# zju3dv/NeuralRecon-W

Measured on NVIDIA H100. Metric: training rays/sec, higher is better.
Workload: dtype bf16 (3-product split forward, plain bf16 backward, fp32 accumulate)

## Files before the change

neuralrecon-w_b200/csrc/engine.cu:

```cuda
#include <stdlib.h>

#include "engine.h"

namespace nrw {

static constexpr float INV_SQRT2 = 0.70710678118654752440f;

struct Carver {
  char* base;
  long long off = 0;
  bool dry;
  void* take(long long bytes) {
    off = round_up(off, 1024);
    void* p = dry ? nullptr : base + off;
    off += bytes;
    return p;
  }
  float* f32(long long n) { return reinterpret_cast<float*>(take(n * 4)); }
  Planes planes(long long rows, int ld, int P) {
    const long long ps = round_up(rows * ld, 512);
    bf16* p = reinterpret_cast<bf16*>(take(ps * P * 2));
    return Planes{p, ps, ld};
  }
};
// ... 51 lines not shown
  c.use_nerf_slot(0);
  c.fwd_cached = false;
  c.ge_acc = cv.f32(4);
  if (with_bwd) {
    const int PB = c.bwd_planes > 0 ? c.bwd_planes : P;
    c.DQ0 = cv.planes(M, 64, PB);
    c.DQodd = cv.planes(M, 512, PB);
    c.DQeven = cv.planes(M, 512, PB);
    c.DQ4 = cv.planes(M, 512, PB);
    c.DA[0] = cv.planes(M, 512, PB);
    c.DA[1] = cv.planes(M, 512, PB);
    c.DFEAT = cv.planes(M, 512, PB);
    c.DQ8f = cv.f32(M * 512);
    for (int l = 0; l < 8; ++l)
      c.DA2[l] = c.aux_bf16 ? side_bf16(reinterpret_cast<bf16*>(cv.take(M * 512 * 2)), 512) : side_f32(cv.f32(M * 512), 512);
    c.dX[0] = cv.planes(M, 256, PB);
    c.dX[1] = cv.planes(M, 256, PB);
    c.dH2 = cv.planes(M, 128, PB);
    c.dH1 = cv.planes(M, 128, PB);
    c.dXF = cv.planes(M, 512, PB);
    c.dNA[0] = cv.planes(M, 128, PB);
    c.dNA[1] = cv.planes(M, 128, PB);
    c.dNF = cv.planes(M, 256, PB);
    c.dNH[0] = cv.planes(M, 256, PB);
    c.dNH[1] = cv.planes(M, 256, PB);
    c.tail = cv.f32(M * 128);
    c.c_dn = cv.f32(M * 3);
    c.c_ddens = cv.f32(M);
    c.gs = cv.f32(c.pm.grad_floats);
  }
  const long long RT = (long long)max_rays * max_T;
  for (int i = 0; i < 2; ++i) { c.gz[i] = cv.f32(RT); c.gsdf[i] = cv.f32(RT); }
  c.gznew = cv.f32(RT);
  c.gsdfnew = cv.f32(RT);
  c.gcdf = cv.f32(RT);
  c.gorder = reinterpret_cast<int32_t*>(cv.f32(RT));
  c.g_pts = cv.f32(RT * 3);
  if (with_bwd) {
    c.g_dsdf = cv.f32(RT);
    c.g_dnrm = cv.f32(RT * 3);
    c.g_drgb = cv.f32(RT * 3);
    c.g_dbga = cv.f32(RT);
    c.g_dbgc = cv.f32(RT * 3);
  }
}

long long workspace_bytes(const nrw_ctx& c0, int chunk_rows, int with_bwd, int max_rays, int max_T, int n_slots_sdf,
                          int n_slots_nerf) {
  nrw_ctx c = c0;
  Carver cv{nullptr, 0, true};
  carve(c, cv, chunk_rows, with_bwd, max_rays, max_T, n_slots_sdf < 1 ? 1 : n_slots_sdf, n_slots_nerf < 1 ? 1 : n_slots_nerf);
  return round_up(cv.off, 1024) + 1024;
}

int carve_workspace(nrw_ctx& c, void* base, long long bytes, int chunk_rows, int with_bwd, int max_rays,
                    int max_T, int n_slots_sdf, int n_slots_nerf, cudaStream_t s) {
  NRW_CHECK(chunk_rows >= 128 && chunk_rows % 128 == 0, NRW_ERR_ARG, "chunk_rows=%d must be a multiple of 128", chunk_rows);
  NRW_CHECK((reinterpret_cast<uintptr_t>(base) & 255) == 0, NRW_ERR_ARG, "workspace must be 256B aligned");
  if (n_slots_sdf < 1) n_slots_sdf = 1;
  if (n_slots_nerf < 1) n_slots_nerf = 1;
  const long long need = workspace_bytes(c, chunk_rows, with_bwd, max_rays, max_T, n_slots_sdf, n_slots_nerf);
  NRW_CHECK(bytes >= need, NRW_ERR_WORKSPACE, "workspace too small: %lld < %lld bytes", bytes, need);
  char* b = reinterpret_cast<char*>((reinterpret_cast<uintptr_t>(base) + 1023) & ~uintptr_t(1023));
  Carver cv{b, 0, false};
  carve(c, cv, chunk_rows, with_bwd, max_rays, max_T, n_slots_sdf, n_slots_nerf);
  NRW_CUDA_OK(cudaMemsetAsync(b, 0, cv.off, s));
  c.Mc = chunk_rows; c.with_bwd = with_bwd; c.max_rays = max_rays; c.max_T = max_T;
  c.bound = true;
  return NRW_OK;
}

static int mm(nrw_ctx& c, Planes A, Planes B, int M, int N, int K, Epi e, cudaStream_t s) {
  GemmDesc g;
  g.A = A; g.B = B; g.n_planes = c.cur_planes; g.M = M; g.N = N; g.K = K; g.mn_major = 0; g.k_slices = 1;
  if (e.out_pl.p) e.n_planes = c.cur_planes;
  g.epi = e;
  return gemm(c.backend, g, s);
}
static int mm_dw(nrw_ctx& c, Planes dY, Planes X, int M, int layer, cudaStream_t s) {
  const PackedLayer& L = c.pm.layers[layer];
  GemmDesc g;
  g.A = dY; g.B = X; g.n_planes = c.cur_planes;
  g.M = L.Np; g.N = L.Kp; g.K = M; g.mn_major = 1;
  const int tiles = cdiv(g.M, 128) * cdiv(g.N, gemm_tc_tile_n(g.N));
  int dev = 0, n_sm = 0;
  NRW_CUDA_OK(cudaGetDevice(&dev));
  NRW_CUDA_OK(cudaDeviceGetAttribute(&n_sm, cudaDevAttrMultiProcessorCount, dev));
  int ks = 2 * n_sm / tiles;
  const int max_ks = M / 512 > 0 ? M / 512 : 1;
  if (ks > max_ks) ks = max_ks;
  if (ks < 1) ks = 1;
  const int kb_total = cdiv(M, 64);
  const int kb_per = cdiv(kb_total, ks);
  ks = cdiv(kb_total, kb_per);
  g.k_slices = ks;
  Epi e;
  e.out_f32 = c.dW(layer); e.ld_f32 = L.Kp; e.atomic = 1;
  g.epi = e;
  return gemm(c.backend, g, s);
}
static int bias_grad(nrw_ctx& c, Planes dY, int M, int layer, cudaStream_t s) {
  return launch_colsum(dY, c.cur_planes, nullptr, 0, M, c.pm.layers[layer].Np, nullptr, c.db(layer), nullptr, s);
}
static void gate_from(nrw_ctx& c, Epi& e, int l, int planes) {
  e.aux_u = c.U[l + 1];
  e.aux_u_planes = planes;
  e.aux_u_scale = (l == 3) ? 1.41421356237309504880f : 1.0f;
}
static Planes rows(Planes P, int r0) { return Planes{P.p + (long long)r0 * P.ld, P.pstride, P.ld}; }

static bool sdf_fused_enabled(const nrw_ctx& c) {
  static const int fused_chain = getenv("NRW_SDF_FUSED") ? atoi(getenv("NRW_SDF_FUSED")) : 1;
  return fused_chain && c.backend == NRW_GEMM_TCGEN05 && c.n_planes == 2;
}
static int sdf_fused_query(nrw_ctx& c, const float* pts, int M, float* sdf, cudaStream_t s) {
  SdfFusedDesc d;
  d.pts = pts; d.sdf = sdf; d.M = M;
  for (int l = 0; l < 8; ++l) { d.W[l] = c.W(L_SDF0 + l); d.bias[l] = c.bias(L_SDF0 + l); }
  d.head_w = c.f_area + c.pm.heads.sdf_w0;
  d.head_b = c.f_area + c.pm.heads.sdf_b0;
  return sdf_fused_forward(d, s);
}

int sdf_chunk_forward(nrw_ctx& c, int M, const float* pts, bool need_normal, bool need_feat, cudaStream_t s) {
  c.cur_planes = c.n_planes;
  const int P = c.n_planes;
  NRW_TRY(launch_sdf_embed(pts, M, P, c.U0, c.U[4], s));
  const float* w0 = c.f_area + c.pm.heads.sdf_w0;
  const float* b0 = c.f_area + c.pm.heads.sdf_b0;
  const bool fused_head = !need_normal && !need_feat && M >= 256 && c.backend == NRW_GEMM_TCGEN05;
  if (fused_head && sdf_fused_enabled(c)) return sdf_fused_query(c, pts, M, c.c_sdf, s);
  for (int l = 0; l < 8; ++l) {
    Epi e;
    e.bias = c.bias(L_SDF0 + l);
    e.act = ACT_SOFTPLUS100;
    if (l == 7 && fused_head) { e.head_w = w0; e.head_partial = c.HP; }
    else e.out_pl = c.U[l + 1];
    if (l == 3) { e.scale = INV_SQRT2; e.n_store = 473; }
    NRW_TRY(mm(c, l == 0 ? c.U0 : c.U[l], c.W(L_SDF0 + l), M, 512, l == 0 ? 64 : 512, e, s));
  }
  if (fused_head) NRW_TRY(launch_sdf_head_sum(c.HP, M, b0, c.c_sdf, s));
  else NRW_TRY(launch_sdf_head(c.U[8], M, w0, b0, c.c_sdf, P, need_normal ? c.G[7] : Planes{nullptr, 0, 0}, s));
  if (need_feat) {
    Epi e;
    e.bias = c.bias(L_SDF8F);
    e.out_pl = c.FEAT;
    NRW_TRY(mm(c, c.U[8], c.W(L_SDF8F), M, 512, 512, e, s));
  }
  if (need_normal) {
    for (int l = 7; l >= 1; --l) {
      Epi e;
      e.out_pre = c.Q[l];
      gate_from(c, e, l - 1, c.n_planes);
      e.out_pl = c.G[l - 1];
      if (l == 4) { e.scale = INV_SQRT2; e.n_store = 473; }
      NRW_TRY(mm(c, c.G[l], c.WT(L_SDF0 + l), M, 512, 512, e, s));
    }
    Epi e;
    e.out_pre = c.Q[0];
    NRW_TRY(mm(c, c.G[0], c.WT(L_SDF0), M, 64, 512, e, s));
    NRW_TRY(launch_sdf_normal(pts, c.Q[0].f32(), c.Q[4].f32(), M, c.c_nrm, s));
  }
  return NRW_OK;
}

int color_chunk_forward(nrw_ctx& c, int M, const float* pts, const float* dirs, const float* a, int rows_per_src,
                        cudaStream_t s) {
  c.cur_planes = c.n_planes;
  const int P = c.n_planes;
  NRW_TRY(launch_color_embed(dirs, a, c.n_a, rows_per_src, pts, c.c_nrm, M, P, c.IN1, c.IN2, s));
  { Epi e; e.bias = c.bias(L_CX); e.out_pl = c.IN1; NRW_TRY(mm(c, c.FEAT, c.W(L_CX), M, 512, 512, e, s)); }
  { Epi e; e.bias = c.bias(L_CS0); e.act = ACT_RELU; e.out_pl = c.H1; NRW_TRY(mm(c, c.IN1, c.W(L_CS0), M, 128, 640, e, s)); }
  { Epi e; e.bias = c.bias(L_CS1); e.act = ACT_RELU; e.out_pl = c.IN2; NRW_TRY(mm(c, c.H1, c.W(L_CS1), M, 128, 128, e, s)); }
  { Epi e; e.bias = c.bias(L_CL0); e.act = ACT_RELU; e.out_pl = c.X[1]; NRW_TRY(mm(c, c.IN2, c.W(L_CL0), M, 256, 192, e, s)); }
  for (int l = 1; l <= 3; ++l) {
    Epi e; e.bias = c.bias(L_CL0 + l); e.act = ACT_RELU; e.out_pl = c.X[l + 1];
    NRW_TRY(mm(c, c.X[l], c.W(L_CL0 + l), M, 256, 256, e, s));
  }
  NRW_TRY(launch_head(3, c.X[4], P, 256, M, c.f_area + c.pm.heads.cl4_w, c.f_area + c.pm.heads.cl4_b, ACT_SIGMOID,
                      nullptr, c.c_rgb, nullptr, s));
  return NRW_OK;
// ... 320 lines not shown
```

neuralrecon-w_b200/csrc/gemm.h:

```cpp
#pragma once
#include "epilogue.cuh"

namespace nrw {

struct GemmDesc {
  Planes A;
  Planes B;
  int n_planes = 1;
  int M = 0, N = 0, K = 0;
  int mn_major = 0;
  int k_slices = 1;
  Epi epi;
};

int gemm_tc(const GemmDesc& g, cudaStream_t stream);
int gemm_simt(const GemmDesc& g, cudaStream_t stream);

inline int gemm(int backend, const GemmDesc& g, cudaStream_t stream) {
  return backend == NRW_GEMM_SIMT ? gemm_simt(g, stream) : gemm_tc(g, stream);
}

inline int n_products(int n_planes) { return n_planes == 1 ? 1 : (n_planes == 2 ? 3 : 6); }

struct SdfFusedDesc {
  const float* pts = nullptr;
  float* sdf = nullptr;
  int M = 0;
  Planes W[8];
  const float* bias[8] = {nullptr, nullptr, nullptr, nullptr, nullptr, nullptr, nullptr, nullptr};
  const float* head_w = nullptr;
  const float* head_b = nullptr;
};
int sdf_fused_forward(const SdfFusedDesc& d, cudaStream_t stream);

long long gemm_tc_launch_count();
inline int gemm_tc_tile_n(int N) { return N <= 64 ? 64 : 128; }
void gemm_tc_set_profile_buffer(unsigned long long* buf);
void gemm_tc_timing_enable(bool on);
int gemm_tc_timing_read(double* ms, double* flops, double* mma_flops, long long* launches, double* bytes);

}
```

neuralrecon-w_b200/csrc/gemm_tc.cu:

```cuda
#include <stdlib.h>

#include <mutex>
#include <unordered_map>
#include <vector>
#include <algorithm>
#include <stdio.h>

#include "gemm.h"
#include "epilogue_fast.cuh"

namespace nrw {

static constexpr int BM = 128;
static constexpr int BK = 64;
static constexpr int RING_BYTES = 192 * 1024;
static constexpr int MAX_STAGES = 8;
static constexpr int N_CONSUMER_WARPS = 8;
static constexpr int N_THREADS = 32 * N_CONSUMER_WARPS + 128;
static constexpr int PRODUCER_REGS = 40, CONSUMER_REGS = 232;
static constexpr int EPI_COLS = 64;
static constexpr int EPI_WG_BYTES = 64 * EPI_COLS * 4;
static constexpr int CS_BYTES = 1024;
static constexpr int BAR_TURN = 4;
static_assert(PRODUCER_REGS * 128 + CONSUMER_REGS * 32 * N_CONSUMER_WARPS <= 65536, "register file");
static constexpr int BAR_BYTES = 256;
static constexpr int SMEM_BYTES = 1024 + RING_BYTES + BAR_BYTES + 2 * EPI_WG_BYTES + CS_BYTES;
static_assert(SMEM_BYTES <= 232448, "dynamic shared memory limit of sm_90");

__device__ __forceinline__ int epi_swz(int r) { return ((r & 1) << 2) | (r & 2) | ((r >> 2) & 1); }

struct TcParams {
  CUtensorMap tmA[3];
  CUtensorMap tmB[3];
  int M, N, K;
  int n_planes;
  int k_slices;
  int m_tiles, n_tiles;
  Epi epi;
  unsigned long long* prof;
};
#define NRW_PROF_T0(cond) const long long _t0 = (cond) ? clock64() : 0
#define NRW_PROF_ADD(cond, slot) \
  if (cond) atomicAdd(&p.prof[blockIdx.x * 16 + (slot)], (unsigned long long)(clock64() - _t0))

__device__ __forceinline__ uint32_t smem_u32(const void* p) {
  return static_cast<uint32_t>(__cvta_generic_to_shared(p));
}
__device__ __forceinline__ void mbar_init(uint32_t bar, uint32_t count) {
  asm volatile("mbarrier.init.shared::cta.b64 [%0], %1;" ::"r"(bar), "r"(count));
}
__device__ __forceinline__ void mbar_wait(uint32_t bar, uint32_t parity) {
  asm volatile(
      "{\n"
      ".reg .pred p;\n"
      "WAIT_LOOP:\n"
      "mbarrier.try_wait.parity.shared::cta.b64 p, [%0], %1;\n"
      "@p bra.uni WAIT_DONE;\n"
      "bra.uni WAIT_LOOP;\n"
      "WAIT_DONE:\n"
      "}\n" ::"r"(bar),
      "r"(parity)
      : "memory");
}
__device__ __forceinline__ void mbar_arrive(uint32_t bar) {
  asm volatile("mbarrier.arrive.shared::cta.b64 _, [%0];" ::"r"(bar) : "memory");
}
__device__ __forceinline__ void mbar_arrive_expect_tx(uint32_t bar, uint32_t bytes) {
  asm volatile("mbarrier.arrive.expect_tx.shared::cta.b64 _, [%0], %1;" ::"r"(bar), "r"(bytes)
               : "memory");
}
__device__ __forceinline__ void tma_load_2d(uint32_t dst, const CUtensorMap* map, uint32_t bar,
                                            int x, int y) {
  asm volatile(
      "cp.async.bulk.tensor.2d.shared::cluster.global.mbarrier::complete_tx::bytes"
      " [%0], [%1, {%3, %4}], [%2];" ::"r"(dst),
      "l"(reinterpret_cast<uint64_t>(map)), "r"(bar), "r"(x), "r"(y)
      : "memory");
}
__device__ __forceinline__ void tma_prefetch_desc(const CUtensorMap* map) {
  asm volatile("prefetch.tensormap [%0];" ::"l"(reinterpret_cast<uint64_t>(map)) : "memory");
}
__device__ __forceinline__ void pdl_wait() { asm volatile("griddepcontrol.wait;" ::: "memory"); }
__device__ __forceinline__ void pdl_launch_dependents() { asm volatile("griddepcontrol.launch_dependents;" ::: "memory"); }
__device__ __forceinline__ void named_bar_sync(int id, int n) { asm volatile("bar.sync %0, %1;" ::"r"(id), "r"(n) : "memory"); }
__device__ __forceinline__ void named_bar_arrive(int id, int n) { asm volatile("bar.arrive %0, %1;" ::"r"(id), "r"(n) : "memory"); }
template <int R>
__device__ __forceinline__ void setmaxnreg_inc() { asm volatile("setmaxnreg.inc.sync.aligned.u32 %0;" ::"n"(R)); }
template <int R>
__device__ __forceinline__ void setmaxnreg_dec() { asm volatile("setmaxnreg.dec.sync.aligned.u32 %0;" ::"n"(R)); }
__device__ __forceinline__ void fence_proxy_async_smem() { asm volatile("fence.proxy.async.shared::cta;" ::: "memory"); }

__device__ __forceinline__ uint64_t make_gdesc(uint32_t saddr, uint32_t lbo_bytes, uint32_t sbo_bytes) {
  uint64_t d = 0;
  d |= (uint64_t)((saddr & 0x3FFFF) >> 4);
  d |= (uint64_t)((lbo_bytes >> 4) & 0x3FFF) << 16;
  d |= (uint64_t)((sbo_bytes >> 4) & 0x3FFF) << 32;
  d |= (uint64_t)1 << 62;
  return d;
}
__device__ __forceinline__ void wgmma_fence() { asm volatile("wgmma.fence.sync.aligned;" ::: "memory"); }
__device__ __forceinline__ void wgmma_commit() { asm volatile("wgmma.commit_group.sync.aligned;" ::: "memory"); }
template <int N>
__device__ __forceinline__ void wgmma_wait() { asm volatile("wgmma.wait_group.sync.aligned %0;" ::"n"(N) : "memory"); }
template <int N>
__device__ __forceinline__ void acc_fence(float (&d)[N]) {
#pragma unroll
  for (int i = 0; i < N; ++i) asm volatile("" : "+f"(d[i])::"memory");
}

template <int BN, int TA, int TB>
__device__ __forceinline__ void wgmma_bf16(float (&d)[BN / 2], uint64_t da, uint64_t db, uint32_t accumulate);

template <>
__device__ __forceinline__ void wgmma_bf16<64, 0, 0>(float (&d)[32], uint64_t da, uint64_t db, uint32_t accumulate) {
  asm volatile(
      "{\n.reg .pred p;\nsetp.ne.b32 p, %34, 0;\n"
      "wgmma.mma_async.sync.aligned.m64n64k16.f32.bf16.bf16 "
      "{%0, %1, %2, %3, %4, %5, %6, %7, %8, %9, %10, %11, %12, %13, %14, %15, %16, %17, %18, %19, %20, %21, %22, %23, %24, %25, "
      "%26, %27, %28, %29, %30, %31}, %32, %33, p, 1, 1, 0, 0;\n}\n"
      : "+f"(d[0]), "+f"(d[1]), "+f"(d[2]), "+f"(d[3]), "+f"(d[4]), "+f"(d[5]), "+f"(d[6]), "+f"(d[7]), "+f"(d[8]), "+f"(d[9]),
        "+f"(d[10]), "+f"(d[11]), "+f"(d[12]), "+f"(d[13]), "+f"(d[14]), "+f"(d[15]), "+f"(d[16]), "+f"(d[17]), "+f"(d[18]),
        "+f"(d[19]), "+f"(d[20]), "+f"(d[21]), "+f"(d[22]), "+f"(d[23]), "+f"(d[24]), "+f"(d[25]), "+f"(d[26]), "+f"(d[27]),
        "+f"(d[28]), "+f"(d[29]), "+f"(d[30]), "+f"(d[31])
      : "l"(da), "l"(db), "r"(accumulate));
}
template <>
__device__ __forceinline__ void wgmma_bf16<64, 1, 1>(float (&d)[32], uint64_t da, uint64_t db, uint32_t accumulate) {
  asm volatile(
      "{\n.reg .pred p;\nsetp.ne.b32 p, %34, 0;\n"
      "wgmma.mma_async.sync.aligned.m64n64k16.f32.bf16.bf16 "
      "{%0, %1, %2, %3, %4, %5, %6, %7, %8, %9, %10, %11, %12, %13, %14, %15, %16, %17, %18, %19, %20, %21, %22, %23, %24, %25, "
      "%26, %27, %28, %29, %30, %31}, %32, %33, p, 1, 1, 1, 1;\n}\n"
      : "+f"(d[0]), "+f"(d[1]), "+f"(d[2]), "+f"(d[3]), "+f"(d[4]), "+f"(d[5]), "+f"(d[6]), "+f"(d[7]), "+f"(d[8]), "+f"(d[9]),
        "+f"(d[10]), "+f"(d[11]), "+f"(d[12]), "+f"(d[13]), "+f"(d[14]), "+f"(d[15]), "+f"(d[16]), "+f"(d[17]), "+f"(d[18]),
        "+f"(d[19]), "+f"(d[20]), "+f"(d[21]), "+f"(d[22]), "+f"(d[23]), "+f"(d[24]), "+f"(d[25]), "+f"(d[26]), "+f"(d[27]),
        "+f"(d[28]), "+f"(d[29]), "+f"(d[30]), "+f"(d[31])
      : "l"(da), "l"(db), "r"(accumulate));
}
#define NRW_WGMMA_N128(TA, TB)                                                                                                          \
  template <>                                                                                                                           \
  __device__ __forceinline__ void wgmma_bf16<128, TA, TB>(float (&d)[64], uint64_t da, uint64_t db, uint32_t accumulate) {              \
    asm volatile(                                                                                                                       \
        "{\n.reg .pred p;\nsetp.ne.b32 p, %66, 0;\n"                                                                                    \
        "wgmma.mma_async.sync.aligned.m64n128k16.f32.bf16.bf16 "                                                                        \
        "{%0, %1, %2, %3, %4, %5, %6, %7, %8, %9, %10, %11, %12, %13, %14, %15, %16, %17, %18, %19, %20, %21, %22, %23, %24, %25, "    \
        "%26, %27, %28, %29, %30, %31, %32, %33, %34, %35, %36, %37, %38, %39, %40, %41, %42, %43, %44, %45, %46, %47, %48, %49, %50, " \
        "%51, %52, %53, %54, %55, %56, %57, %58, %59, %60, %61, %62, %63}, %64, %65, p, 1, 1, " #TA ", " #TB ";\n}\n"                   \
        : "+f"(d[0]), "+f"(d[1]), "+f"(d[2]), "+f"(d[3]), "+f"(d[4]), "+f"(d[5]), "+f"(d[6]), "+f"(d[7]), "+f"(d[8]), "+f"(d[9]),     \
          "+f"(d[10]), "+f"(d[11]), "+f"(d[12]), "+f"(d[13]), "+f"(d[14]), "+f"(d[15]), "+f"(d[16]), "+f"(d[17]), "+f"(d[18]),        \
          "+f"(d[19]), "+f"(d[20]), "+f"(d[21]), "+f"(d[22]), "+f"(d[23]), "+f"(d[24]), "+f"(d[25]), "+f"(d[26]), "+f"(d[27]),        \
          "+f"(d[28]), "+f"(d[29]), "+f"(d[30]), "+f"(d[31]), "+f"(d[32]), "+f"(d[33]), "+f"(d[34]), "+f"(d[35]), "+f"(d[36]),        \
          "+f"(d[37]), "+f"(d[38]), "+f"(d[39]), "+f"(d[40]), "+f"(d[41]), "+f"(d[42]), "+f"(d[43]), "+f"(d[44]), "+f"(d[45]),        \
          "+f"(d[46]), "+f"(d[47]), "+f"(d[48]), "+f"(d[49]), "+f"(d[50]), "+f"(d[51]), "+f"(d[52]), "+f"(d[53]), "+f"(d[54]),        \
          "+f"(d[55]), "+f"(d[56]), "+f"(d[57]), "+f"(d[58]), "+f"(d[59]), "+f"(d[60]), "+f"(d[61]), "+f"(d[62]), "+f"(d[63])         \
        : "l"(da), "l"(db), "r"(accumulate));                                                                                           \
  }
NRW_WGMMA_N128(0, 0)
NRW_WGMMA_N128(1, 1)
#undef NRW_WGMMA_N128


template <int BN, int MN_MAJOR, int EK>
__global__ void __launch_bounds__(N_THREADS, 1) gemm_tc_kernel(const __grid_constant__ TcParams p) {
  static_assert(BN == 64 || BN == 128, "wgmma tile width");
  constexpr int A_TILE = BM * BK * 2;
  constexpr int B_TILE = BN * BK * 2;
  constexpr int WG_A = 64 * BK * 2;
  extern __shared__ uint8_t smem_raw[];
  uint8_t* smem = smem_raw + ((1024u - (smem_u32(smem_raw) & 1023u)) & 1023u);
  const int P = p.n_planes;
  const int stage_bytes = P * (A_TILE + B_TILE);
  int stages = RING_BYTES / stage_bytes;
  if (stages > MAX_STAGES) stages = MAX_STAGES;
  uint64_t* bars = reinterpret_cast<uint64_t*>(smem + RING_BYTES);
  const uint32_t bar_full = smem_u32(bars), bar_empty = smem_u32(bars + MAX_STAGES);
  float* epi_buf = reinterpret_cast<float*>(smem + RING_BYTES + BAR_BYTES);
  float* cs_buf = reinterpret_cast<float*>(smem + RING_BYTES + BAR_BYTES + 2 * EPI_WG_BYTES);
  const int warp = threadIdx.x >> 5, lane = threadIdx.x & 31;
  const long long t_kernel0 = clock64();

  if (warp == N_CONSUMER_WARPS && lane == 0) {
    for (int i = 0; i < P; ++i) {
      tma_prefetch_desc(&p.tmA[i]);
      tma_prefetch_desc(&p.tmB[i]);
    }
    for (int i = 0; i < MAX_STAGES; ++i) {
      mbar_init(bar_full + 8 * i, 1);
      mbar_init(bar_empty + 8 * i, 4);
    }
    asm volatile("fence.mbarrier_init.release.cluster;" ::: "memory");
  }
  if (threadIdx.x < 256) cs_buf[threadIdx.x] = 0.0f;
  __syncthreads();
  pdl_wait();
  pdl_launch_dependents();

  const int kb_total = (p.K + BK - 1) / BK;
  const int kb_per = (kb_total + p.k_slices - 1) / p.k_slices;
  const int n_items = p.m_tiles * p.n_tiles * p.k_slices;
  const int n_prod = (P == 1) ? 1 : (P == 2 ? 3 : 6);

  if (warp >= N_CONSUMER_WARPS) {
    setmaxnreg_dec<PRODUCER_REGS>();
    if (warp == N_CONSUMER_WARPS && lane == 0) {
      int s = 0;
      uint32_t ph = 0;
      for (int item = blockIdx.x; item < n_items; item += gridDim.x) {
        const int ks = item % p.k_slices;
        const int t = item / p.k_slices;
        const int n0 = (t % p.n_tiles) * BN, m0 = (t / p.n_tiles) * BM;
        const int kb0 = ks * kb_per, kb1 = min(kb_total, kb0 + kb_per);
        for (int kb = kb0; kb < kb1; ++kb) {
          {
            NRW_PROF_T0(p.prof != nullptr);
            mbar_wait(bar_empty + 8 * s, ph ^ 1);
            NRW_PROF_ADD(p.prof != nullptr, 0);
          }
          mbar_arrive_expect_tx(bar_full + 8 * s, stage_bytes);
          const uint32_t sa = smem_u32(smem + s * stage_bytes);
          const uint32_t sb = sa + P * A_TILE;
          for (int pl = 0; pl < P; ++pl) {
            if (MN_MAJOR == 0) {
              tma_load_2d(sa + pl * A_TILE, &p.tmA[pl], bar_full + 8 * s, kb * BK, m0);
              tma_load_2d(sb + pl * B_TILE, &p.tmB[pl], bar_full + 8 * s, kb * BK, n0);
            } else {
#pragma unroll
              for (int sl = 0; sl < BM / 64; ++sl)
                tma_load_2d(sa + pl * A_TILE + sl * (64 * BK * 2), &p.tmA[pl], bar_full + 8 * s,
                            m0 + 64 * sl, kb * BK);
#pragma unroll
              for (int sl = 0; sl < BN / 64; ++sl)
                tma_load_2d(sb + pl * B_TILE + sl * (64 * BK * 2), &p.tmB[pl], bar_full + 8 * s,
                            n0 + 64 * sl, kb * BK);
            }
          }
          if (++s == stages) { s = 0; ph ^= 1; }
        }
      }
    }
  } else {
    setmaxnreg_inc<CONSUMER_REGS>();
    const int wg = warp >> 2, wi = warp & 3;
    const uint32_t smem0 = smem_u32(smem);
    constexpr uint32_t LBO = MN_MAJOR ? (64 * BK * 2) : 16;
    constexpr uint32_t SBO = 1024;
    constexpr uint32_t KSTEP = MN_MAJOR ? (16 * 128) : 32;
    const uint64_t desc_hi = make_gdesc(0, LBO, SBO);
    float* stage_tile = epi_buf + wg * (EPI_WG_BYTES / 4);
    const bool use_cs = p.epi.colsum != nullptr && !p.epi.atomic;
    float* cs_wg = cs_buf + 128 * wg;
    const int ctid = threadIdx.x & 127;
    const bool prof = p.prof != nullptr && wi == 0 && lane == 0;
    const int po = 8 * wg;
    int cs_n0 = -1;
    int s = 0;
    uint32_t ph = 0;
    for (int j = 0; blockIdx.x + j * gridDim.x < n_items; ++j) {
      const int item = blockIdx.x + j * gridDim.x;
      const int ks = item % p.k_slices;
      const int t = item / p.k_slices;
      const int n0 = (t % p.n_tiles) * BN, m0 = (t / p.n_tiles) * BM;
      const int kb0 = ks * kb_per, kb1 = min(kb_total, kb0 + kb_per);
      if ((j & 1) != wg) {
        for (int kb = kb0; kb < kb1; ++kb)
          if (++s == stages) { s = 0; ph ^= 1; }
        continue;
      }
      if (use_cs && n0 != cs_n0) {
        if (cs_n0 >= 0) colsum_flush(cs_wg, p.epi.colsum, cs_n0, min(min(p.N, p.epi.n_store) - cs_n0, BN), ctid, 128, 2 + wg);
        cs_n0 = n0;
      }
      float acc[2][BN / 2];
#pragma unroll
      for (int h = 0; h < 2; ++h)
#pragma unroll
        for (int i = 0; i < BN / 2; ++i) acc[h][i] = 0.0f;
      if (j > 0) {
        NRW_PROF_T0(prof);
        named_bar_sync(BAR_TURN + wg, 256);
        NRW_PROF_ADD(prof, 3 + po);
      }
      int prev_s = -1;
      for (int kb = kb0; kb < kb1; ++kb) {
        {
          NRW_PROF_T0(prof);
          mbar_wait(bar_full + 8 * s, ph);
          NRW_PROF_ADD(prof, 1 + po);
        }
        const uint32_t sa = smem0 + s * stage_bytes;
        const uint32_t sb = smem0 + s * stage_bytes + P * A_TILE;
        wgmma_fence();
        for (int pr = 0; pr < n_prod; ++pr) {
          const int q = 4 * (n_prod - 1 - pr);
          const uint32_t pa = (0x021010u >> q) & 0xFu, pb = (0x201100u >> q) & 0xFu;
          const uint64_t da = desc_hi | (uint64_t)(((sa + pa * A_TILE) & 0x3FFFFu) >> 4);
          const uint64_t db = desc_hi | (uint64_t)(((sb + pb * B_TILE) & 0x3FFFFu) >> 4);
#pragma unroll
          for (int k = 0; k < BK / 16; ++k)
#pragma unroll
            for (int h = 0; h < 2; ++h)
              wgmma_bf16<BN, MN_MAJOR, MN_MAJOR>(acc[h], da + ((h * WG_A + k * KSTEP) >> 4), db + ((k * KSTEP) >> 4), 1u);
        }
        wgmma_commit();
        acc_fence(acc[0]);
        acc_fence(acc[1]);
        if (prev_s >= 0) {
          wgmma_wait<1>();
          acc_fence(acc[0]);
          acc_fence(acc[1]);
          if (lane == 0) mbar_arrive(bar_empty + 8 * prev_s);
        }
        prev_s = s;
        if (++s == stages) { s = 0; ph ^= 1; }
      }
      if (item + gridDim.x < n_items) named_bar_arrive(BAR_TURN + (wg ^ 1), 256);
      wgmma_wait<0>();
      acc_fence(acc[0]);
      acc_fence(acc[1]);
      if (prev_s >= 0 && lane == 0) mbar_arrive(bar_empty + 8 * prev_s);
      if (kb1 <= kb0) continue;
      NRW_PROF_T0(prof);
// ... 145 lines not shown
  cudaLaunchAttribute attr[1];
  attr[0].id = cudaLaunchAttributeProgrammaticStreamSerialization;
  attr[0].val.programmaticStreamSerializationAllowed = 1;
  cfg.attrs = attr;
  cfg.numAttrs = pdl ? 1 : 0;
  return cudaLaunchKernelEx(&cfg, kernel, p);
}

template <int BN, int MN, int EK>
static int launch(const TcParams& p, int n_sm, int dev, cudaStream_t stream) {
  static bool attr_set[MAX_DEV] = {false};
  if (!attr_set[dev]) {
    NRW_CUDA_OK((cudaFuncSetAttribute(gemm_tc_kernel<BN, MN, EK>, cudaFuncAttributeMaxDynamicSharedMemorySize, SMEM_BYTES)));
    attr_set[dev] = true;
  }
  const int items = p.m_tiles * p.n_tiles * p.k_slices;
  const int grid = items < n_sm ? items : n_sm;
  NRW_CUDA_OK((launch_gemm(gemm_tc_kernel<BN, MN, EK>, grid, N_THREADS, stream, p)));
  NRW_LAUNCH_OK();
  ++g_tc_launches;
  return NRW_OK;
}

static int gemm_tc_impl(const GemmDesc& g, cudaStream_t stream);

struct TimedLaunch { cudaEvent_t e0, e1; double flops; double mma_flops; int M, N, K, P, mn, ks; unsigned epi; double bytes; };
static std::vector<TimedLaunch> g_timed;
static std::vector<cudaEvent_t> g_event_pool;
static bool g_timing_on = false;
void gemm_tc_timing_enable(bool on) { g_timing_on = on; }
static cudaEvent_t get_event() {
  if (!g_event_pool.empty()) { cudaEvent_t e = g_event_pool.back(); g_event_pool.pop_back(); return e; }
  cudaEvent_t e;
  cudaEventCreate(&e);
  return e;
}
int gemm_tc_timing_read(double* ms, double* flops, double* mma_flops, long long* launches, double* bytes) {
  double t = 0, f = 0, mf = 0, by = 0;
  FILE* dump = getenv("NRW_GEMM_TIMING_DUMP") ? fopen(getenv("NRW_GEMM_TIMING_DUMP"), "a") : nullptr;
  for (auto& L : g_timed) {
    NRW_CUDA_OK(cudaEventSynchronize(L.e1));
    float dt = 0;
    NRW_CUDA_OK(cudaEventElapsedTime(&dt, L.e0, L.e1));
    t += dt; f += L.flops; mf += L.mma_flops; by += L.bytes;
    g_event_pool.push_back(L.e0); g_event_pool.push_back(L.e1);
    if (dump) fprintf(dump, "%d,%d,%d,%d,%d,%d,%u,%.0f,%.4f\n", L.M, L.N, L.K, L.P, L.mn, L.ks, L.epi, L.bytes, dt);
  }
  if (dump) fclose(dump);
  *ms = t; *flops = f; *mma_flops = mf; *launches = (long long)g_timed.size();
  if (bytes) *bytes = by;
  g_timed.clear();
  return NRW_OK;
}

int gemm_tc(const GemmDesc& g, cudaStream_t stream) {
  if (!g_timing_on) return gemm_tc_impl(g, stream);
  TimedLaunch L;
  L.e0 = get_event(); L.e1 = get_event();
  L.flops = 2.0 * g.M * g.N * g.K;
  L.mma_flops = L.flops * n_products(g.n_planes);
  L.M = g.M; L.N = g.N; L.K = g.K; L.P = g.n_planes; L.mn = g.mn_major; L.ks = g.k_slices;
  const Epi& e = g.epi;
  const int q_bytes = e.aux_q_bcast ? 0 : e.aux_q.elem_bytes();
  L.epi = (e.out_pre ? 1u : 0u) | (e.out_f32 ? 2u : 0u) | (e.out2 ? 4u : 0u) | (e.n_planes ? 8u : 0u) | (e.aux_u.p ? 16u : 0u) |
          (q_bytes ? 32u : 0u) | (e.aux_add ? 64u : 0u) | (e.aux_relu ? 128u : 0u) | (e.atomic ? 256u : 0u) | (e.colsum ? 512u : 0u);
  const double mn = (double)g.M * (double)std::min(g.N, e.n_store);
  L.bytes = 2.0 * g.n_planes * ((double)g.M * g.K + (double)g.N * g.K) + (double)e.out_pre.elem_bytes() * g.M * g.N +
            mn * (4.0 * (e.out_f32 ? 1 : 0) + e.out2.elem_bytes() + q_bytes + e.aux_add.elem_bytes() + 2.0 * e.n_planes +
                  (e.aux_relu ? 2.0 : 0.0) + (e.aux_u.p ? 2.0 * e.aux_u_planes : 0.0));
  NRW_CUDA_OK(cudaEventRecord(L.e0, stream));
  const int rc = gemm_tc_impl(g, stream);
  NRW_CUDA_OK(cudaEventRecord(L.e1, stream));
  g_timed.push_back(L);
  return rc;
}
static int gemm_tc_impl(const GemmDesc& g, cudaStream_t stream) {
  NRW_CHECK(g.M > 0 && g.N > 0 && g.K > 0, NRW_ERR_ARG, "gemm_tc: empty problem %d %d %d", g.M, g.N, g.K);
  NRW_CHECK(g.n_planes >= 1 && g.n_planes <= 3, NRW_ERR_ARG, "gemm_tc: n_planes=%d", g.n_planes);
  NRW_CHECK(g.k_slices == 1 || g.epi.atomic, NRW_ERR_ARG, "gemm_tc: split-K needs an atomic epilogue");
  static int n_sm_dev[MAX_DEV] = {0};
  const int dev = current_device();
  if (!n_sm_dev[dev]) NRW_CUDA_OK(cudaDeviceGetAttribute(&n_sm_dev[dev], cudaDevAttrMultiProcessorCount, dev));
  const int n_sm = n_sm_dev[dev];
  const int BN = g.N <= 64 ? 64 : 128;
  TcParams p;
  memset(&p, 0, sizeof(p));
  p.M = g.M; p.N = g.N; p.K = g.K; p.n_planes = g.n_planes; p.k_slices = g.k_slices;
  p.m_tiles = cdiv(g.M, BM); p.n_tiles = cdiv(g.N, BN);
  p.epi = g.epi;
  p.prof = g_prof_ptr;
  for (int pl = 0; pl < g.n_planes; ++pl) {
    if (!g.mn_major) {
      NRW_CHECK(g.K % BK == 0, NRW_ERR_ARG, "gemm_tc: K=%d must be a multiple of %d (pad the operand)", g.K, BK);
      NRW_TRY(make_map(&p.tmA[pl], g.A.plane(pl), g.K, g.M, g.A.ld, BK, BM));
      NRW_TRY(make_map(&p.tmB[pl], g.B.plane(pl), g.K, g.N, g.B.ld, BK, BN));
    } else {
      NRW_TRY(make_map(&p.tmA[pl], g.A.plane(pl), g.M, g.K, g.A.ld, 64, BK));
      NRW_TRY(make_map(&p.tmB[pl], g.B.plane(pl), g.N, g.K, g.B.ld, 64, BK));
    }
  }
  const int ek = g.mn_major ? EK_GENERIC : pick_epi_kind(g.epi);
  NRW_CHECK(ek >= 0 && (ek != EK_FWD_HEAD || g.N == 512), NRW_ERR_ARG,
            "gemm_tc: the fused SDF-head epilogue needs N = 512, bias + softplus and no other output");
  if (g.mn_major) return BN == 64 ? launch<64, 1, EK_GENERIC>(p, n_sm, dev, stream) : launch<128, 1, EK_GENERIC>(p, n_sm, dev, stream);
  if (BN == 64) return launch<64, 0, EK_GENERIC>(p, n_sm, dev, stream);
  switch (ek) {
    case EK_FWD_SOFTPLUS: return launch<128, 0, EK_FWD_SOFTPLUS>(p, n_sm, dev, stream);
    case EK_FWD_RELU: return launch<128, 0, EK_FWD_RELU>(p, n_sm, dev, stream);
    case EK_FWD_NONE: return launch<128, 0, EK_FWD_NONE>(p, n_sm, dev, stream);
    case EK_FWD_HEAD: return launch<128, 0, EK_FWD_HEAD>(p, n_sm, dev, stream);
    case EK_GATE_FWD: return launch<128, 0, EK_GATE_FWD>(p, n_sm, dev, stream);
    case EK_TANGENT: return launch<128, 0, EK_TANGENT>(p, n_sm, dev, stream);
    case EK_REVERSE: return launch<128, 0, EK_REVERSE>(p, n_sm, dev, stream);
    case EK_RELU_BWD: return launch<128, 0, EK_RELU_BWD>(p, n_sm, dev, stream);
    default: return launch<128, 0, EK_GENERIC>(p, n_sm, dev, stream);
  }
}


static constexpr int FZ_ROWS = 64;
static constexpr int FZ_APLANE = FZ_ROWS * 512 * 2;
static constexpr int FZ_A = 2 * FZ_APLANE;
static constexpr int FZ_WG = 4;
static constexpr int FZ_WSTAGE = 64 * BK * 2;
static constexpr int FZ_NST = 3;
static constexpr int FZ_BAR = FZ_A + FZ_WG * FZ_NST * FZ_WSTAGE;
static constexpr int FZ_SMEM = 1024 + FZ_BAR + 256;
static constexpr int FZ_THREADS = 128 * FZ_WG;
static constexpr int FZ_POS_PER_TILE = 4 * (1 + 7 * 8);
static_assert(FZ_SMEM <= 232448, "dynamic shared memory limit of sm_90");

struct SdfFusedParams {
  CUtensorMap tmW[8][2];
  const float* bias[8];
  const float* head_w;
  const float* head_b;
  const float* pts;
  float* sdf;
  int M, n_tiles;
};

__device__ __forceinline__ float pe6_feature(const float (&x)[3], int f) {
  if (f < 3) return x[f];
  const int k = (f - 3) / 6, wi = (f - 3) % 6, c = wi % 3;
  float sn, cs;
  sincosf(x[c] * (float)(1 << k), &sn, &cs);
  return wi < 3 ? sn : cs;
}

__global__ void __launch_bounds__(FZ_THREADS, 1) sdf_fused_kernel(const __grid_constant__ SdfFusedParams p) {
  extern __shared__ uint8_t smem_raw[];
  uint8_t* smem = smem_raw + ((1024u - (smem_u32(smem_raw) & 1023u)) & 1023u);
  uint64_t* bars = reinterpret_cast<uint64_t*>(smem + FZ_BAR);
  const uint32_t w_full = smem_u32(bars);
  const int warp = threadIdx.x >> 5, lane = threadIdx.x & 31;
  const uint32_t smem0 = smem_u32(smem);
  const int g = warp >> 2, wi = warp & 3, et = threadIdx.x;
  const bool loader = wi == 0 && lane == 0;

  if (et == 0) {
    for (int l = 0; l < 8; ++l) { tma_prefetch_desc(&p.tmW[l][0]); tma_prefetch_desc(&p.tmW[l][1]); }
    for (int i = 0; i < FZ_WG * FZ_NST; ++i) mbar_init(w_full + 8 * i, 1);
    asm volatile("fence.mbarrier_init.release.cluster;" ::: "memory");
  }
  __syncthreads();
  pdl_wait();
  pdl_launch_dependents();

  auto load = [&](int pos) {
    const int tile = blockIdx.x + (pos / FZ_POS_PER_TILE) * gridDim.x;
    if (tile >= p.n_tiles) return;
    const int q = pos % FZ_POS_PER_TILE;
    const int l = q < 4 ? 0 : 1 + (q - 4) / 32, r = q < 4 ? q : (q - 4) % 32;
    const int kb = r >> 2, u = r & 3;
    const uint32_t st = g * FZ_NST + pos % FZ_NST;
    mbar_arrive_expect_tx(w_full + 8 * st, FZ_WSTAGE);
    tma_load_2d(smem0 + FZ_A + st * FZ_WSTAGE, &p.tmW[l][(u & 1) ? 0 : 1], w_full + 8 * st, kb * BK, 128 * g + 64 * (u >> 1));
  };
  if (loader)
    for (int i = 0; i < FZ_NST; ++i) load(i);

  {
    const int r0 = 16 * wi + (lane >> 2), c0 = 2 * (lane & 3);
    const uint64_t desc_hi = make_gdesc(0, 16, 1024);
    float* part = reinterpret_cast<float*>(smem);
    int pos = 0;
// ... 192 lines not shown
```

Measured before the change: 36520.

## Add cooperative 256x128 weight-gradient GEMM tile with vector red.add epilogue

Adds a cooperative schedule for the MN-major weight-gradient GEMM: both consumer warpgroups share one B tile across a 256-row A tile, with the producer loading four A slices per stage. The epilogue writes accumulators straight to global memory with red.global.add.v2.f32 instead of staging through shared memory. The goal is to halve B-tile traffic per output, cut tile count and atomic overhead in split-K dW. It only applies to single-plane backward GEMMs (plain bf16 backward) with M>=256 and N>64. The split-K heuristic now uses the larger tile, which gives fewer tiles and more k-slices, so there are more atomic adds.

```diff
diff --git a/neuralrecon-w_b200/csrc/engine.cu b/neuralrecon-w_b200/csrc/engine.cu
--- a/neuralrecon-w_b200/csrc/engine.cu
+++ b/neuralrecon-w_b200/csrc/engine.cu
@@ -157,7 +157,10 @@
   GemmDesc g;
   g.A = dY; g.B = X; g.n_planes = c.cur_planes;
   g.M = L.Np; g.N = L.Kp; g.K = M; g.mn_major = 1;
-  const int tiles = cdiv(g.M, 128) * cdiv(g.N, gemm_tc_tile_n(g.N));
+  Epi e;
+  e.out_f32 = c.dW(layer); e.ld_f32 = L.Kp; e.atomic = 1;
+  g.epi = e;
+  const int tiles = cdiv(g.M, gemm_tc_tile_m(g)) * cdiv(g.N, gemm_tc_tile_n(g.N));
   int dev = 0, n_sm = 0;
   NRW_CUDA_OK(cudaGetDevice(&dev));
   NRW_CUDA_OK(cudaDeviceGetAttribute(&n_sm, cudaDevAttrMultiProcessorCount, dev));
@@ -169,9 +172,6 @@
   const int kb_per = cdiv(kb_total, ks);
   ks = cdiv(kb_total, kb_per);
   g.k_slices = ks;
-  Epi e;
-  e.out_f32 = c.dW(layer); e.ld_f32 = L.Kp; e.atomic = 1;
-  g.epi = e;
   return gemm(c.backend, g, s);
 }
 static int bias_grad(nrw_ctx& c, Planes dY, int M, int layer, cudaStream_t s) {
diff --git a/neuralrecon-w_b200/csrc/gemm.h b/neuralrecon-w_b200/csrc/gemm.h
--- a/neuralrecon-w_b200/csrc/gemm.h
+++ b/neuralrecon-w_b200/csrc/gemm.h
@@ -35,6 +35,12 @@
 
 long long gemm_tc_launch_count();
 inline int gemm_tc_tile_n(int N) { return N <= 64 ? 64 : 128; }
+inline bool gemm_tc_dw_coop(const GemmDesc& g) {
+  const Epi& e = g.epi;
+  return g.mn_major && g.n_planes == 1 && g.M >= 256 && g.N > 64 && e.atomic && e.out_f32 && e.ld_f32 % 2 == 0 &&
+         (reinterpret_cast<uintptr_t>(e.out_f32) & 7) == 0 && !e.bias && !e.rowvec && !e.out_pre && !e.colsum;
+}
+inline int gemm_tc_tile_m(const GemmDesc& g) { return gemm_tc_dw_coop(g) ? 256 : 128; }
 void gemm_tc_set_profile_buffer(unsigned long long* buf);
 void gemm_tc_timing_enable(bool on);
 int gemm_tc_timing_read(double* ms, double* flops, double* mma_flops, long long* launches, double* bytes);
diff --git a/neuralrecon-w_b200/csrc/gemm_tc.cu b/neuralrecon-w_b200/csrc/gemm_tc.cu
--- a/neuralrecon-w_b200/csrc/gemm_tc.cu
+++ b/neuralrecon-w_b200/csrc/gemm_tc.cu
@@ -22,6 +22,7 @@
 static constexpr int EPI_WG_BYTES = 64 * EPI_COLS * 4;
 static constexpr int CS_BYTES = 1024;
 static constexpr int BAR_TURN = 4;
+static constexpr int MN_COOP = 2;
 static_assert(PRODUCER_REGS * 128 + CONSUMER_REGS * 32 * N_CONSUMER_WARPS <= 65536, "register file");
 static constexpr int BAR_BYTES = 256;
 static constexpr int SMEM_BYTES = 1024 + RING_BYTES + BAR_BYTES + 2 * EPI_WG_BYTES + CS_BYTES;
@@ -89,6 +90,9 @@
 template <int R>
 __device__ __forceinline__ void setmaxnreg_dec() { asm volatile("setmaxnreg.dec.sync.aligned.u32 %0;" ::"n"(R)); }
 __device__ __forceinline__ void fence_proxy_async_smem() { asm volatile("fence.proxy.async.shared::cta;" ::: "memory"); }
+__device__ __forceinline__ void red_add_v2(float* out, float a, float b) {
+  asm volatile("red.global.add.v2.f32 [%0], {%1, %2};" ::"l"(out), "f"(a), "f"(b) : "memory");
+}
 
 __device__ __forceinline__ uint64_t make_gdesc(uint32_t saddr, uint32_t lbo_bytes, uint32_t sbo_bytes) {
   uint64_t d = 0;
@@ -163,7 +167,10 @@
 template <int BN, int MN_MAJOR, int EK>
 __global__ void __launch_bounds__(N_THREADS, 1) gemm_tc_kernel(const __grid_constant__ TcParams p) {
   static_assert(BN == 64 || BN == 128, "wgmma tile width");
-  constexpr int A_TILE = BM * BK * 2;
+  constexpr bool COOP = MN_MAJOR == MN_COOP;
+  static_assert(!COOP || (BN == 128 && EK == EK_GENERIC), "the cooperative schedule is the 256 x 128 weight-gradient tile");
+  constexpr int TM = COOP ? 2 * BM : BM;
+  constexpr int A_TILE = TM * BK * 2;
   constexpr int B_TILE = BN * BK * 2;
   constexpr int WG_A = 64 * BK * 2;
   extern __shared__ uint8_t smem_raw[];
@@ -186,7 +193,7 @@
     }
     for (int i = 0; i < MAX_STAGES; ++i) {
       mbar_init(bar_full + 8 * i, 1);
-      mbar_init(bar_empty + 8 * i, 4);
+      mbar_init(bar_empty + 8 * i, COOP ? 8 : 4);
     }
     asm volatile("fence.mbarrier_init.release.cluster;" ::: "memory");
   }
@@ -208,7 +215,7 @@
       for (int item = blockIdx.x; item < n_items; item += gridDim.x) {
         const int ks = item % p.k_slices;
         const int t = item / p.k_slices;
-        const int n0 = (t % p.n_tiles) * BN, m0 = (t / p.n_tiles) * BM;
+        const int n0 = (t % p.n_tiles) * BN, m0 = (t / p.n_tiles) * TM;
         const int kb0 = ks * kb_per, kb1 = min(kb_total, kb0 + kb_per);
         for (int kb = kb0; kb < kb1; ++kb) {
           {
@@ -225,7 +232,7 @@
               tma_load_2d(sb + pl * B_TILE, &p.tmB[pl], bar_full + 8 * s, kb * BK, n0);
             } else {
 #pragma unroll
-              for (int sl = 0; sl < BM / 64; ++sl)
+              for (int sl = 0; sl < TM / 64; ++sl)
                 tma_load_2d(sa + pl * A_TILE + sl * (64 * BK * 2), &p.tmA[pl], bar_full + 8 * s,
                             m0 + 64 * sl, kb * BK);
 #pragma unroll
@@ -237,6 +244,85 @@
           if (++s == stages) { s = 0; ph ^= 1; }
         }
       }
+    }
+  } else if constexpr (COOP) {
+    setmaxnreg_inc<CONSUMER_REGS>();
+    const int wg = warp >> 2, wi = warp & 3;
+    const uint32_t smem0 = smem_u32(smem);
+    const uint64_t desc_hi = make_gdesc(0, 64 * BK * 2, 1024);
+    constexpr uint32_t KSTEP = 16 * 128;
+    const bool prof = p.prof != nullptr && wi == 0 && lane == 0;
+    const int po = 8 * wg;
+    const int n_lim = min(p.N, p.epi.n_store);
+    int s = 0;
+    uint32_t ph = 0;
+    for (int item = blockIdx.x; item < n_items; item += gridDim.x) {
+      const int ks = item % p.k_slices;
+      const int t = item / p.k_slices;
+      const int n0 = (t % p.n_tiles) * BN, m0 = (t / p.n_tiles) * TM;
+      const int kb0 = ks * kb_per, kb1 = min(kb_total, kb0 + kb_per);
+      float acc[2][BN / 2];
+#pragma unroll
+      for (int h = 0; h < 2; ++h)
+#pragma unroll
+        for (int i = 0; i < BN / 2; ++i) acc[h][i] = 0.0f;
+      int prev_s = -1;
+      for (int kb = kb0; kb < kb1; ++kb) {
+        {
+          NRW_PROF_T0(prof);
+          mbar_wait(bar_full + 8 * s, ph);
+          NRW_PROF_ADD(prof, 1 + po);
+        }
+        const uint32_t sa = smem0 + s * stage_bytes;
+        const uint32_t sb = smem0 + s * stage_bytes + P * A_TILE;
+        wgmma_fence();
+        for (int pr = 0; pr < n_prod; ++pr) {
+          const int q = 4 * (n_prod - 1 - pr);
+          const uint32_t pa = (0x021010u >> q) & 0xFu, pb = (0x201100u >> q) & 0xFu;
+          const uint64_t da = desc_hi | (uint64_t)(((sa + pa * A_TILE + 2 * wg * WG_A) & 0x3FFFFu) >> 4);
+          const uint64_t db = desc_hi | (uint64_t)(((sb + pb * B_TILE) & 0x3FFFFu) >> 4);
+#pragma unroll
+          for (int k = 0; k < BK / 16; ++k)
+#pragma unroll
+            for (int h = 0; h < 2; ++h)
+              wgmma_bf16<BN, 1, 1>(acc[h], da + ((h * WG_A + k * KSTEP) >> 4), db + ((k * KSTEP) >> 4), 1u);
+        }
+        wgmma_commit();
+        acc_fence(acc[0]);
+        acc_fence(acc[1]);
+        if (prev_s >= 0) {
+          wgmma_wait<1>();
+          acc_fence(acc[0]);
+          acc_fence(acc[1]);
+          if (lane == 0) mbar_arrive(bar_empty + 8 * prev_s);
+        }
+        prev_s = s;
+        if (++s == stages) { s = 0; ph ^= 1; }
+      }
+      wgmma_wait<0>();
+      acc_fence(acc[0]);
+      acc_fence(acc[1]);
+      if (prev_s >= 0 && lane == 0) mbar_arrive(bar_empty + 8 * prev_s);
+      if (kb1 <= kb0) continue;
+      NRW_PROF_T0(prof);
+      if (prof) atomicAdd(&p.prof[blockIdx.x * 16 + 6 + po], 1ull);
+      const int c0 = n0 + 2 * (lane & 3);
+#pragma unroll
+      for (int h = 0; h < 2; ++h)
+#pragma unroll
+        for (int r8 = 0; r8 < 2; ++r8) {
+          const int row = m0 + 128 * wg + 64 * h + 16 * wi + (lane >> 2) + 8 * r8;
+          if (row >= p.M) continue;
+          float* dst = p.epi.out_f32 + (long long)row * p.epi.ld_f32;
+#pragma unroll
+          for (int j = 0; j < BN / 8; ++j) {
+            const int c = c0 + 8 * j;
+            const float x0 = acc[h][4 * j + 2 * r8] * p.epi.scale, x1 = acc[h][4 * j + 2 * r8 + 1] * p.epi.scale;
+            if (c + 1 < n_lim) red_add_v2(dst + c, x0, x1);
+            else if (c < n_lim) atomicAdd(dst + c, x0);
+          }
+        }
+      NRW_PROF_ADD(prof, 4 + po);
     }
   } else {
     setmaxnreg_inc<CONSUMER_REGS>();
@@ -548,11 +634,12 @@
   const int dev = current_device();
   if (!n_sm_dev[dev]) NRW_CUDA_OK(cudaDeviceGetAttribute(&n_sm_dev[dev], cudaDevAttrMultiProcessorCount, dev));
   const int n_sm = n_sm_dev[dev];
-  const int BN = g.N <= 64 ? 64 : 128;
+  const int BN = gemm_tc_tile_n(g.N);
+  const bool coop = gemm_tc_dw_coop(g);
   TcParams p;
   memset(&p, 0, sizeof(p));
   p.M = g.M; p.N = g.N; p.K = g.K; p.n_planes = g.n_planes; p.k_slices = g.k_slices;
-  p.m_tiles = cdiv(g.M, BM); p.n_tiles = cdiv(g.N, BN);
+  p.m_tiles = cdiv(g.M, gemm_tc_tile_m(g)); p.n_tiles = cdiv(g.N, BN);
   p.epi = g.epi;
   p.prof = g_prof_ptr;
   for (int pl = 0; pl < g.n_planes; ++pl) {
@@ -568,6 +655,7 @@
   const int ek = g.mn_major ? EK_GENERIC : pick_epi_kind(g.epi);
   NRW_CHECK(ek >= 0 && (ek != EK_FWD_HEAD || g.N == 512), NRW_ERR_ARG,
             "gemm_tc: the fused SDF-head epilogue needs N = 512, bias + softplus and no other output");
+  if (coop) return launch<128, MN_COOP, EK_GENERIC>(p, n_sm, dev, stream);
   if (g.mn_major) return BN == 64 ? launch<64, 1, EK_GENERIC>(p, n_sm, dev, stream) : launch<128, 1, EK_GENERIC>(p, n_sm, dev, stream);
   if (BN == 64) return launch<64, 0, EK_GENERIC>(p, n_sm, dev, stream);
   switch (ek) {
```

Result: faster. 38240, median of 6 (+4.7%).
